# castorini/howl

Hardware: AMD Instinct MI355X
Metric: utterances/sec/node (res8 end-to-end training step, 1s@16kHz, 40-mel) (higher is better)
Workload: dtype f32; 1 GPU; res8 training step (frontend+fwd+xent+bwd+AdamW), 512 x 1 s utterances per GPU, 12 labels -- BASELINE configs[2] per-GPU share: res8 GSC-12, 512 x 1 s per GPU (4096 over 8); global_batch=512, samples_per_utterance=16000, labels=12, parallelism=single, frontend=eval

## Files before the change

### howl_amd/csrc/res8.hip

```cpp
#include "howl_common.hip.h"
#include "../../include/howl_hip.h"

namespace {

struct HowlPtrs6 {
    float* p[6];
};
constexpr int MAX_WINDOWS = 64;
struct HowlWinRows {
    int lo[MAX_WINDOWS], hi[MAX_WINDOWS];
};
struct HowlBnBuffers {
    float* running_mean;
    float* running_var;
    long long* num_batches;
};
struct BnFold {
    const float* part;
    int nparts;
    double count;
    float* stats_out;
    HowlBnBuffers bn;
};

// ... 1646 lines not shown
#pragma unroll
        for (int nt = 0; nt < 3; ++nt) {
            const int tap = 4 * ks + g, c = 16 * nt + n;
            bw[ks][nt] = (tap < 9 && c < NMAP) ? w0[c * 9 + tap] : 0.0f;
        }
    int aoff[3];
#pragma unroll
    for (int ks = 0; ks < 3; ++ks) {
        const int tap = min(4 * ks + g, 8);
        aoff[ks] = (tap / 3) * pitch + tap % 3 + (n & 7) + (n >> 3) * 3 * pitch;
    }
    for (int i = tid; i < 3 * pitch + 16; i += C0M_THREADS) tin[(T + 2) * pitch + i] = 0.0f;
    for (int item = blockIdx.x; item < B * slices; item += nconv) {
        const int b = item / slices, sl = item - b * slices;
        const int ph0 = (sl * H) / slices, ph1 = ((sl + 1) * H) / slices;
        __syncthreads();
        const int clip = b / nwin, wi = b - clip * nwin;
        const int t0 = EXACT ? wi * win_step : min(wi * win_step, win_last);
        load_feat_tile<EXACT>(tin, feat + (long)clip * sb + (long)t0 * st, 0, st, sm, 0, T, M, tid, C0M_THREADS, -t0, win_last - t0);
        __syncthreads();
        constexpr int NJ = 5 * NS;
        for (int u = wave; u < NJ * ((ph1 - ph0 + 1) / 2); u += C0M_THREADS / 64) {
            const int pp = u / NJ, j8 = u - NJ * pp;
            const float* rowp = tin + 3 * (ph0 + 2 * pp) * pitch + 8 * j8;
            {
                f32x4 acc[3][3];
#pragma unroll
                for (int tl = 0; tl < 3; ++tl)
#pragma unroll
                    for (int nt = 0; nt < 3; ++nt) acc[tl][nt] = {0.0f, 0.0f, 0.0f, 0.0f};
#pragma unroll
                for (int tl = 0; tl < 3; ++tl)
#pragma unroll
                    for (int ks = 0; ks < 3; ++ks) {
                        const float a = rowp[aoff[ks] + tl * pitch];
#pragma unroll
                        for (int nt = 0; nt < 3; ++nt)
                            acc[tl][nt] = __builtin_amdgcn_mfma_f32_16x16x4f32(a, bw[ks][nt], acc[tl][nt], 0, 0, 0);
                    }
                const int pw = 2 * j8 + (g & 1), ph = ph0 + 2 * pp + (g >> 1);
#pragma unroll
                for (int nt = 0; nt < 3; ++nt) {
                    float sum = 0.0f;
                    unsigned bits = 0;
#pragma unroll
                    for (int tl = 0; tl < 3; ++tl)
#pragma unroll
                        for (int r = 0; r < 4; ++r) {
                            const int rb = max(__float_as_int(acc[tl][nt][r]), 0);
                            sum += __int_as_float(rb);
                            bits |= min((unsigned)rb, 1u) << (4 * tl + r);
                        }
                    const int c = 16 * nt + n;
                    if (ph < ph1 && c < NMAP) {
                        const int strip = NS > 1 ? pw / PW : 0;
                        const size_t o = (((size_t)b * NS + strip) * NMAP + c) * P + (size_t)ph * PW + (pw - strip * PW);
                        s0[o] = sum * (1.0f / 12.0f);
                        if (mask0 != nullptr) mask0[o] = (unsigned short)bits;
                    }
                }
            }
        }
    }
}

constexpr int C0G_WAVES = 15, C0G_THREADS = 64 * C0G_WAVES, C0G_CPW = NMAP / C0G_WAVES;
static_assert(C0G_CPW * C0G_WAVES == NMAP, "channels split evenly over the waves");

__device__ __forceinline__ void load_patch(float (&x)[5][6], const float* tin, int pitch, int ph, int pw) {
    const float* base = tin + 3 * ph * pitch + 4 * pw;
#pragma unroll
    for (int r = 0; r < 5; ++r) {
        const float4 a = *reinterpret_cast<const float4*>(base + r * pitch);
        const float2 c = *reinterpret_cast<const float2*>(base + r * pitch + 4);
        x[r][0] = a.x, x[r][1] = a.y, x[r][2] = a.z, x[r][3] = a.w, x[r][4] = c.x, x[r][5] = c.y;
    }
}

template <int NS = 1, bool EXACT = false>
__global__ __launch_bounds__(C0G_THREADS) void conv0_wgrad_valu_kernel(const float* __restrict__ feat, long sb, long st, long sm,
                                                                      const unsigned short* __restrict__ mask0,
                                                                      const float* __restrict__ ga, const float* __restrict__ gb,
                                                                      float* __restrict__ part, int B, int T, int M, int H,
                                                                      int slices, StripGeom sg, int t_total) {
    HIP_DYNAMIC_SHARED(float, lds)
    float* tin = lds;
    const int tid = threadIdx.x, lane = tid & 63;
    const int wave = __builtin_amdgcn_readfirstlane(tid >> 6);
    const int pitch = M + 4;
    const int P = H * PW;
    float acc[C0G_CPW][9];
#pragma unroll
    for (int j = 0; j < C0G_CPW; ++j)
#pragma unroll
        for (int t = 0; t < 9; ++t) acc[j][t] = 0.0f;
    const int nrs = EXACT ? sg.nr : 1;
    for (int item = blockIdx.x; item < B * nrs * NS * slices; item += gridDim.x) {
        const int vb = item / slices, sl = item - vb * slices;
        const int vq = NS > 1 ? vb / NS : vb, strip = NS > 1 ? vb - vq * NS : 0;
        const int b = EXACT ? vq / nrs : vq, rs = EXACT ? vq - b * nrs : 0;
        const int Pv = (EXACT && rs == nrs - 1) ? sg.hv_last * PW : P;
        const int cell0 = (sl * Pv) / slices, cell1 = ((sl + 1) * Pv) / slices;
        __syncthreads();
        if constexpr (EXACT)
            load_feat_tile<true>(tin, feat + (long)rs * T * st, sb, st, sm, b, T, M, tid, C0G_THREADS, -rs * T, t_total - rs * T);
        else
            load_feat_tile(tin, feat, sb, st, sm, b, T, M, tid, C0G_THREADS);
        __syncthreads();
        const float* gab = ga + ((size_t)vb * NMAP + C0G_CPW * wave) * P;
        const float* gbb = gb != nullptr ? gb + ((size_t)vb * NMAP + C0G_CPW * wave) * P : nullptr;
        const unsigned short* mb = mask0 + ((size_t)vb * NMAP + C0G_CPW * wave) * P;
        for (int cb = cell0; cb < cell1; cb += 64) {
            const int cell = cb + lane;
            const bool valid = cell < cell1;
            const unsigned cc = (unsigned)(valid ? cell : cell1 - 1);
            float gv[C0G_CPW];
            unsigned mv[C0G_CPW];
#pragma unroll
            for (int j = 0; j < C0G_CPW; ++j) {
                const unsigned o = (unsigned)(j * P) + cc;
                gv[j] = gab[o] + (gbb != nullptr ? gbb[o] : 0.0f);
                mv[j] = mb[o];
            }
            const int ph = (int)cc / PW, pw = (int)cc - ph * PW;
            float x[5][6];
            load_patch(x, tin, pitch, ph, pw + strip * PW);
#pragma unroll
            for (int j = 0; j < C0G_CPW; ++j) {
                const int gbits = valid ? __float_as_int(gv[j] * (1.0f / 12.0f)) : 0;
#pragma unroll
                for (int tl = 0; tl < 3; ++tl)
#pragma unroll
                    for (int fl = 0; fl < 4; ++fl) {
                        const int k = 4 * tl + fl;
                        const int sel = ((int)(mv[j] << (31 - k))) >> 31;
                        const float dy = __int_as_float(sel & gbits);
#pragma unroll
                        for (int tap = 0; tap < 9; ++tap) acc[j][tap] = fmaf(dy, x[tl + tap / 3][fl + tap % 3], acc[j][tap]);
                    }
            }
        }
    }
#pragma unroll
    for (int j = 0; j < C0G_CPW; ++j)
#pragma unroll
        for (int t = 0; t < 9; ++t) {
            const float v = wave_sum_rows(acc[j][t]);
            if (lane == 0) part[(size_t)blockIdx.x * NMAP * 9 + (C0G_CPW * wave + j) * 9 + t] = v;
        }
}

constexpr int HEAD_XC = 64;
constexpr int HEAD_THREADS = 768, HEAD_PARTS = 16;
__global__ __launch_bounds__(HEAD_THREADS) void head_fwd_kernel(const float* __restrict__ s6, const float* __restrict__ stats,
                                                       const float* __restrict__ wout, const float* __restrict__ bout,
                                                       float* __restrict__ pooled, float* __restrict__ logits, int B,
                                                       int P, int C, const long long* __restrict__ labels,
                                                       float* __restrict__ nll, float* __restrict__ dlogits,
                                                       float* __restrict__ dpool, float inv_batch,
                                                       const float* __restrict__ pool, int npg, int npg_used, BnFold fold,
                                                       int ns ) {
    __shared__ float lp[CP];
    __shared__ float ll[HEAD_XC], dl[HEAD_XC], lse_s;
    __shared__ float lst[2 * CP];
    __shared__ float lw[HEAD_XC * NMAP];
    __shared__ float lparts[HEAD_PARTS][CP];
    const int tid = threadIdx.x, lane = tid & 63, wave = tid >> 6;
    const bool w_in_lds = C <= HEAD_XC;
    if (w_in_lds)
        for (int i = tid; i < C * NMAP; i += HEAD_THREADS) lw[i] = wout[i];
    if (fold.part != nullptr) {
        const int c8 = lane >> 3;
        for (int w0 = wave; w0 < CP / 4; w0 += HEAD_THREADS / 64) {
            const int c = 4 * w0 + (c8 & 3);
            const double sm = fold_part_column(fold.part, part_stride(fold.nparts), fold.nparts, (c8 < 4 ? 0 : CP) + c, lane);
            const double q = __shfl_xor(sm, 32);
            if (c8 < 4 && (lane & 7) == 0) {
                const double mean = sm / fold.count;
                double var = q / fold.count - mean * mean;
                var = var < 0.0 ? 0.0 : var;
                const float fm = (c < NMAP) ? (float)mean : 0.0f;
                const float fr = (c < NMAP) ? (float)(1.0 / sqrt(var + (double)BN_EPS)) : 0.0f;
                lst[c] = fm;
                lst[CP + c] = fr;
                if (blockIdx.x == 0) {
                    fold.stats_out[c] = fm;
                    fold.stats_out[CP + c] = fr;
                    if (c < NMAP && fold.bn.running_mean != nullptr) {
                        const double unbiased = fold.count > 1.0 ? var * fold.count / (fold.count - 1.0) : var;
                        fold.bn.running_mean[c] = (1.0f - BN_MOMENTUM) * fold.bn.running_mean[c] + BN_MOMENTUM * (float)mean;
                        fold.bn.running_var[c] = (1.0f - BN_MOMENTUM) * fold.bn.running_var[c] + BN_MOMENTUM * (float)unbiased;
                    }
                    if (c == 0 && fold.bn.num_batches != nullptr) fold.bn.num_batches[0] += 1;
                }
            }
        }
    } else if (tid < 2 * CP) {
        lst[tid] = stats[tid];
    }
    __syncthreads();
    for (int b = blockIdx.x; b < B; b += gridDim.x) {
        __syncthreads();
        if (pool != nullptr) {
            const int nparts = ns * npg_used;
            const int pc = tid % CP, pk = tid / CP;
            float acc = 0.0f;
            for (int k0 = 0; k0 < nparts; k0 += HEAD_PARTS) {
                const int k = k0 + pk;
                if (k < nparts) {
                    const int sgi = k / npg_used, g = k - sgi * npg_used;
                    lparts[pk][pc] = pool[(((size_t)b * ns + sgi) * npg + g) * CP + pc];
                }
                __syncthreads();
                if (tid < CP) {
                    const int n = nparts - k0 < HEAD_PARTS ? nparts - k0 : HEAD_PARTS;
                    for (int j = 0; j < n; ++j) acc += lparts[j][tid];
                }
                __syncthreads();
            }
            if (tid < CP) {
                const float v = tid < NMAP ? (acc / (float)P - lst[tid]) * lst[CP + tid] : 0.0f;
                lp[tid] = v;
                pooled[(size_t)b * CP + tid] = v;
            }
        } else if (wave < 4)
        for (int c0 = wave; c0 < CP; c0 += 12) {
            float a8[3][8];
#pragma unroll
            for (int u = 0; u < 3; ++u) {
                const int c = c0 + 4 * u < NMAP ? c0 + 4 * u : NMAP - 1;
                const float* src = s6 + ((size_t)b * NMAP + c) * P;
#pragma unroll
                for (int j = 0; j < 8; ++j) a8[u][j] = src[min(lane + 64 * j, P - 1)];
            }
#pragma unroll
            for (int u = 0; u < 3; ++u) {
                const int c = c0 + 4 * u;
#pragma unroll
                for (int j = 0; j < 8; ++j) a8[u][j] = (lane + 64 * j < P) ? fabsf(a8[u][j]) : 0.0f;
                float acc = ((a8[u][0] + a8[u][1]) + (a8[u][2] + a8[u][3])) + ((a8[u][4] + a8[u][5]) + (a8[u][6] + a8[u][7]));
                acc = wave_sum(acc);
                const float v = c < NMAP ? (acc / (float)P - lst[c]) * lst[CP + c] : 0.0f;
                if (lane == 0 && c < CP) {
                    lp[c] = v;
                    pooled[(size_t)b * CP + c] = v;
                }
            }
        }
        __syncthreads();
        for (int k = tid; k < C; k += HEAD_THREADS) {
            float acc = bout[k];
            if (w_in_lds)
                for (int c = 0; c < NMAP; ++c) acc = fmaf(lw[k * NMAP + c], lp[c], acc);
            else
                for (int c = 0; c < NMAP; ++c) acc = fmaf(wout[k * NMAP + c], lp[c], acc);
            logits[(size_t)b * C + k] = acc;
            if (labels != nullptr) ll[k] = acc;
        }
        if (labels == nullptr) continue;
        __syncthreads();
        const int y = (int)labels[b];
        if (tid == 0) {
            float mx = ll[0];
            for (int k = 1; k < C; ++k) mx = fmaxf(mx, ll[k]);
            float se = 0.0f;
            for (int k = 0; k < C; ++k) se += expf(ll[k] - mx);
            const float lse = mx + logf(se);
            lse_s = lse;
            nll[b] = lse - ll[y];
        }
        __syncthreads();
        if (tid < C) {
            const float d = (expf(ll[tid] - lse_s) - (tid == y ? 1.0f : 0.0f)) * inv_batch;
            dl[tid] = d;
            dlogits[(size_t)b * C + tid] = d;
        }
        __syncthreads();
        if (tid < CP) {
            float acc = 0.0f;
            if (tid < NMAP)
                for (int k = 0; k < C; ++k) acc = fmaf(dl[k], lw[k * NMAP + tid], acc);
            dpool[(size_t)b * CP + tid] = acc;
        }
    }
}

__global__ __launch_bounds__(256) void head_fwd_windows_kernel(const float* __restrict__ s6, const float* __restrict__ stats,
                                                               const float* __restrict__ wout, const float* __restrict__ bout,
                                                               float* __restrict__ logits, int B, int nwin, int Hw,
                                                               HowlWinRows rows, float inv_count, int C, int ns) {
    __shared__ float lp[CP];
    const int tid = threadIdx.x, lane = tid & 63, wave = tid >> 6;
    const int Pw = Hw * PW;
    for (int b = blockIdx.x; b < B; b += gridDim.x) {
        __syncthreads();
        for (int c = wave; c < CP; c += 4) {
            float acc = 0.0f;
            if (c < NMAP) {
                for (int w = 0; w < nwin * ns; ++w) {
                    const float* src = s6 + ((size_t)(b * nwin * ns + w) * NMAP + c) * Pw;
                    for (int i = rows.lo[w / ns] * PW + lane; i < rows.hi[w / ns] * PW; i += 64) acc += fabsf(src[i]);
                }
            }
            acc = wave_sum(acc);
            if (lane == 0) lp[c] = c < NMAP ? (acc * inv_count - stats[c]) * stats[CP + c] : 0.0f;
        }
        __syncthreads();
        for (int k = tid; k < C; k += 256) {
            float acc = bout[k];
            for (int c = 0; c < NMAP; ++c) acc = fmaf(wout[k * NMAP + c], lp[c], acc);
            logits[(size_t)b * C + k] = acc;
        }
    }
}

__global__ void head_bwd_pool_kernel(const float* __restrict__ dlogits, const float* __restrict__ wout,
                                     float* __restrict__ dpool, int B, int C) {
    const int idx = blockIdx.x * blockDim.x + threadIdx.x;
    if (idx >= B * CP) return;
    const int b = idx / CP, c = idx - b * CP;
    float acc = 0.0f;
    if (c < NMAP)
        for (int k = 0; k < C; ++k) acc = fmaf(dlogits[(size_t)b * C + k], wout[k * NMAP + c], acc);
    dpool[idx] = acc;
}

__global__ __launch_bounds__(1024) void head_bwd_param_kernel(const float* __restrict__ dlogits,
                                                              const float* __restrict__ pooled,
                                                              const float* __restrict__ dpool, float* __restrict__ dwout,
                                                              float* __restrict__ dbout, float* __restrict__ m12, int B,
                                                              int C, int P, const float* __restrict__ nll,
                                                              float* __restrict__ loss) {
    __shared__ double red[2][16][64];
    if ((int)blockIdx.x == C + 1) {
        double acc = 0.0;
        for (int b = threadIdx.x; b < B; b += 1024) acc += (double)nll[b];
        acc = wave_sum_d(acc);
        if ((threadIdx.x & 63) == 0) red[0][threadIdx.x >> 6][0] = acc;
        __syncthreads();
        if (threadIdx.x == 0) {
            double tot = 0.0;
            for (int w = 0; w < 16; ++w) tot += red[0][w][0];
            loss[0] = (float)(tot / (double)B);
        }
        return;
    }
    const int k = blockIdx.x, c = threadIdx.x & 63, bg = threadIdx.x >> 6;
    double a0 = 0.0, a1 = 0.0;
    constexpr int HR = 16;
    const int cc = c < CP ? c : CP - 1;
    if (k < C) {
        for (int b = bg; b < B; b += 16 * HR) {
            float d[HR], pv[HR];
#pragma unroll
            for (int j = 0; j < HR; ++j) {
                const int bb = b + 16 * j < B ? b + 16 * j : B - 1;
                d[j] = dlogits[(size_t)bb * C + k];
                pv[j] = pooled[(size_t)bb * CP + cc];
            }
#pragma unroll
            for (int j = 0; j < HR; ++j) {
                const bool ok = b + 16 * j < B;
                a1 += ok ? (double)d[j] : 0.0;
                a0 += (ok && c < CP) ? (double)d[j] * (double)pv[j] : 0.0;
            }
        }
    } else if (c < CP) {
        for (int b = bg; b < B; b += 16 * HR) {
            float d[HR], pv[HR];
#pragma unroll
            for (int j = 0; j < HR; ++j) {
                const int bb = b + 16 * j < B ? b + 16 * j : B - 1;
                d[j] = dpool[(size_t)bb * CP + c];
                pv[j] = pooled[(size_t)bb * CP + c];
            }
#pragma unroll
            for (int j = 0; j < HR; ++j) {
                const bool ok = b + 16 * j < B;
                a0 += ok ? (double)d[j] : 0.0;
                a1 += ok ? (double)d[j] * (double)pv[j] : 0.0;
            }
        }
    }
    red[0][bg][c] = a0;
    red[1][bg][c] = a1;
    __syncthreads();
    if (bg != 0) return;
    double s0 = 0.0, s1 = 0.0;
    for (int g = 0; g < 16; ++g) {
        s0 += red[0][g][c];
        s1 += red[1][g][c];
    }
    if (k < C) {
        if (c < NMAP) dwout[k * NMAP + c] = (float)s0;
        if (c == 0) dbout[k] = (float)s1;
    } else if (c < CP) {
        const double n = (double)B * (double)P;
        m12[c] = (float)(s0 / n);
        m12[CP + c] = (float)(s1 / n);
    }
}

__global__ __launch_bounds__(1024) void xent_kernel(const float* __restrict__ logits, const long long* __restrict__ labels,
                                                    int B, int C, float* __restrict__ loss, float* __restrict__ dlogits) {
    __shared__ double red[16];
    double acc = 0.0;
    const float invB = 1.0f / (float)B;
    constexpr int XC = 32;
    for (int b = threadIdx.x; b < B; b += 1024) {
        const float* row = logits + (size_t)b * C;
        const int y = (int)labels[b];
        if (C <= XC) {
            float v[XC];
#pragma unroll
            for (int k = 0; k < XC; ++k) v[k] = row[k < C ? k : C - 1];
            float mx = v[0];
#pragma unroll
            for (int k = 1; k < XC; ++k) mx = k < C ? fmaxf(mx, v[k]) : mx;
            float se = 0.0f;
#pragma unroll
            for (int k = 0; k < XC; ++k) se += k < C ? expf(v[k] - mx) : 0.0f;
            const float lse = mx + logf(se);
            float vy = v[0];
#pragma unroll
            for (int k = 1; k < XC; ++k) vy = k == y ? v[k] : vy;
            acc += (double)(lse - vy);
            if (dlogits != nullptr) {
#pragma unroll
                for (int k = 0; k < XC; ++k)
                    if (k < C) dlogits[(size_t)b * C + k] = (expf(v[k] - lse) - (k == y ? 1.0f : 0.0f)) * invB;
            }
            continue;
        }
        float mx = row[0];
        for (int k = 1; k < C; ++k) mx = fmaxf(mx, row[k]);
        float se = 0.0f;
        for (int k = 0; k < C; ++k) se += expf(row[k] - mx);
        const float lse = mx + logf(se);
        acc += (double)(lse - row[y]);
        if (dlogits != nullptr)
            for (int k = 0; k < C; ++k)
                dlogits[(size_t)b * C + k] = (expf(row[k] - lse) - (k == y ? 1.0f : 0.0f)) * invB;
    }
    acc = wave_sum_d(acc);
    if ((threadIdx.x & 63) == 0) red[threadIdx.x >> 6] = acc;
    __syncthreads();
    if (threadIdx.x == 0) {
        double tot = 0.0;
        for (int w = 0; w < 16; ++w) tot += red[w];
        loss[0] = (float)(tot / (double)B);
    }
}

__global__ void adamw_kernel(float* __restrict__ p, const float* __restrict__ g, float* __restrict__ m,
                             float* __restrict__ v, size_t n, HowlAdamWCoef c) {
    for (size_t i = (size_t)blockIdx.x * blockDim.x + threadIdx.x; i < n; i += (size_t)gridDim.x * blockDim.x)
        howl_adamw_element(p, m, v, i, g[i], c);
}

}

namespace {

size_t conv0_tile_floats(int T, int M) { return (size_t)(T + 2) * (M + 4) + 3 * (M + 4) + 16; }
size_t conv_lds_bytes(int H, bool own_rows) {
    return (size_t)(3 * KSTEPS * 64 + tile_floats(H, own_rows) + 4 * CP + 12 * 2 * 16) * sizeof(float);
}
size_t wgrad_lds_bytes(int H) { return (size_t)(tile_floats_z(H) + tile_floats_x(H) + 6 * CP) * sizeof(float); }

struct Ws {
    float* wp_fwd;
    float* wp_bwd;
    float* part;
    float* part2;
    float* stats;
    float* m12;
    float* dpool;
    float* pool;
    float* bufa;
    float* bufb;
    float* dz;
    float* dz2;
    float* dsa;
    float* dsb;
    float* wpart;
    float* c0part;
};

size_t ws_layout(Ws* w, char* base, int B, int H, int G, int cus, size_t* fwd_eval_bytes) {
    size_t off = 0;
    auto take = [&](size_t floats) {
        float* p = base ? reinterpret_cast<float*>(base + off) : nullptr;
        off += ((floats * sizeof(float) + 255) / 256) * 256;
        return p;
    };
    const size_t act = (size_t)B * NMAP * H * PW;
    w->wp_fwd = take((size_t)6 * 3 * KSTEPS * 64);
    w->wp_bwd = take((size_t)6 * 3 * KSTEPS * 64);
    const int max_parts = G > cus ? G : cus;
    w->part = take((size_t)part_stride(max_parts) * 2 * CP);
    w->part2 = take((size_t)part_stride(max_parts) * 2 * CP);
    w->stats = take((size_t)6 * 2 * CP);
    w->m12 = take(2 * CP);
    w->dpool = take((size_t)B * CP);
    w->pool = take((size_t)B * 16 * CP);
    *fwd_eval_bytes = off;
    w->bufa = take(act);
    w->bufb = take(act);
    w->dz = take(act);
    w->dz2 = take(act);
    w->dsa = take(act);
    w->dsb = take(act);
    w->wpart = take((size_t)6 * G * CP * WNCOL);
    w->c0part = take((size_t)max_parts * NMAP * 9);
    return off;
}

int mel_strips(int M) { return M == 40 ? 1 : (M == 80 ? 2 : 0); }
int even_grid(int g, int strips) { return strips > 1 ? ((g & ~1) > 2 ? (g & ~1) : 2) : g; }
int launch_blocks(int nblk, int per_group) { return 8 * per_group * ((nblk + 7) / 8); }
int conv_slices(int nblk, int H, int budget) {
    const int ntiles = (H * PW + 15) / 16;
    for (int sl = 4; sl > 1; sl >>= 1)
        if (nblk * sl <= budget && 4 * sl <= ntiles) return sl;
    return 1;
}
void pair_slices(int nblk, int H, int cus, int* sd, int* sw) {
    const int ntiles = (H * PW + 15) / 16;
    const int opts[3][2] = {{4, 2}, {2, 2}, {2, 1}};
    *sd = *sw = 1;
    for (const auto& o : opts)
        if (nblk * (o[0] + o[1]) <= cus && 4 * o[0] <= ntiles) {
            *sd = o[0];
            *sw = o[1];
            return;
        }
}
int conv0_slices(int B, int cus) {
    const int sl = cus / (B > 0 ? B : 1);
    return sl < 1 ? 1 : (sl > 8 ? 8 : sl);
}
bool env_off(const char* name) {
    const char* e = getenv(name);
    return e != nullptr && e[0] == '0';
}

constexpr int WIN_H = MAX_H, WIN_MARGIN = 7, WIN_STEP = WIN_H - 2 * WIN_MARGIN;
int long_windows(int H) { return H <= WIN_H ? 1 : (H - WIN_H + WIN_STEP - 1) / WIN_STEP + 1; }

struct Res8Plan {
    int B, T, M, ns, nr, Hs, hv_last, Bv, halo;
    StripGeom sg;
    int P, Pt;
    bool slicing, merged, fused;
    int G, SL;
    size_t lds_conv;
    int Bw, Tw, S0, G0, c0_nwin, c0_step, c0_last;
    bool c0_exact;
    size_t lds_conv0;
    int Gh, SD, SW, ew_grid;
    bool fold_in_pair;
    size_t wpart_stride, lds_wgrad, lds_pair;
    int S0w, G0w;
    size_t lds_conv0w;
    size_t saved_floats, train_bytes, eval_bytes;
    size_t long_map_bytes, long_bytes;
    Ws ws;
};

void plan_launches(Res8Plan& p, bool slice_conv0, char* ws_base) {
    const int cus = howl_num_cus(), H = p.Hs;
    p.P = H * PW;
    p.Pt = (p.T / 3) * PW * p.ns;
    p.saved_floats = (size_t)p.Bv * NMAP * p.P;
    p.slicing = !env_off("HOWL_RES8_SLICES");
    p.merged = !env_off("HOWL_RES8_BWD_PAIR");
    p.fused = p.halo != 0 || !env_off("HOWL_RES8_BWD_FUSED");

    p.G = even_grid(p.Bv < cus ? p.Bv : cus, p.ns);
    p.SL = p.halo == 0 && p.slicing ? conv_slices(p.G, H, cus) : 1;
    p.lds_conv = conv_lds_bytes(H, p.halo == 2);
    p.S0 = slice_conv0 && p.slicing ? conv0_slices(p.Bw, cus) : 1;
    p.G0 = p.Bw * p.S0 < 2 * cus ? p.Bw * p.S0 : 2 * cus;
    p.lds_conv0 = conv0_tile_floats(p.Tw, p.M) * sizeof(float);

    const int half = cus / 2 > 0 ? cus / 2 : 1;
    p.Gh = even_grid(p.Bv < half ? p.Bv : half, p.ns);
    p.SD = p.SW = 1;
    if (p.halo == 0 && p.slicing) pair_slices(p.Gh, H, cus, &p.SD, &p.SW);
    p.fold_in_pair = p.Gh * p.SD >= 64;
    p.wpart_stride = (size_t)p.Gh * CP * WNCOL;
    p.lds_wgrad = wgrad_lds_bytes(H);
    p.lds_pair = p.lds_conv > p.lds_wgrad ? p.lds_conv : p.lds_wgrad;
    const size_t quads = (p.saved_floats / 4 + BRB_THREADS - 1) / BRB_THREADS;
    p.ew_grid = quads < 1 ? 1 : (quads > (size_t)(2 * cus) ? 2 * cus : (int)quads);
    p.S0w = p.slicing ? conv0_slices(p.Bv, cus) : 1;
    p.G0w = p.Bv * p.S0w < cus ? p.Bv * p.S0w : cus;
    p.lds_conv0w = ((size_t)(p.Tw + 2) * (p.M + 4) + 16) * sizeof(float);

    p.train_bytes = ws_layout(&p.ws, ws_base, p.Bv, H, p.G, cus, &p.eval_bytes);
}

Res8Plan res8_plan(int B, int T, int M, void* ws = nullptr) {
    Res8Plan p{};
    const int H = T / 3;
    p.B = B, p.T = T, p.M = M;
    p.ns = mel_strips(M) > 0 ? mel_strips(M) : 1;
    p.nr = H <= MAX_H ? 1 : (H + MAX_H - 1) / MAX_H;
    p.Hs = (H + p.nr - 1) / p.nr;
    p.hv_last = H - (p.nr - 1) * p.Hs;
    p.Bv = B * p.nr * p.ns;
    p.halo = p.nr > 1 ? 2 : (p.ns > 1 ? 1 : 0);
    p.sg = StripGeom{p.nr, p.ns, p.hv_last};
    p.c0_exact = p.halo == 2;
    p.Bw = B * p.nr;
    p.Tw = p.c0_exact ? 3 * p.Hs : T;
    p.c0_nwin = p.c0_exact ? p.nr : 1;
    p.c0_step = p.c0_exact ? 3 * p.Hs : 0;
    p.c0_last = p.c0_exact ? T : 0;
    plan_launches(p, true, static_cast<char*>(ws));
    return p;
}

Res8Plan res8_long_plan(int B, int T, int M, void* ws = nullptr) {
    Res8Plan p{};
    const int H = T / 3, nw = long_windows(H);
    p.B = B, p.T = T, p.M = M;
    p.ns = mel_strips(M) > 0 ? mel_strips(M) : 1;
    p.nr = 1, p.Hs = p.hv_last = WIN_H;
    p.Bv = B * nw * p.ns;
    p.halo = p.ns > 1 ? 1 : 0;
    p.sg = StripGeom{1, 1, 0};
    p.Bw = B * nw;
    p.Tw = 3 * WIN_H + T % 3;
    p.c0_nwin = nw, p.c0_step = 3 * WIN_STEP, p.c0_last = 3 * (H - WIN_H);
    static_assert((6 * 2 * CP * sizeof(float)) % 256 == 0, "statistics block keeps the 256-byte alignment");
    p.long_map_bytes = ((size_t)p.Bv * NMAP * WIN_H * PW * sizeof(float) + 255) / 256 * 256;
    const size_t front = 3 * p.long_map_bytes + 6 * 2 * CP * sizeof(float) + 256;
    plan_launches(p, false, ws ? static_cast<char*>(ws) + front : nullptr);
    p.long_bytes = front + p.train_bytes;
    return p;
}

int check_workspace(const char* who, size_t have, size_t need) {
    if (have >= need) return HOWL_OK;
    howl_set_error("%s: workspace %zu < %zu bytes", who, have, need);
    return HOWL_E_WORKSPACE;
}
template <class T>
HowlPtrs6 ptrs6(T* const (&a)[6]) {
    HowlPtrs6 r;
    for (int i = 0; i < 6; ++i) r.p[i] = const_cast<float*>(a[i]);
    return r;
}
StageCfg plain_tile(const float* t) { return StageCfg{t, nullptr, nullptr, nullptr, nullptr, 0.0f, false, false, false}; }

template <auto Kernel>
void raise_lds_limit(size_t lds) {
    static thread_local size_t granted[16] = {};
    howl_raise_lds(reinterpret_cast<const void*>(Kernel), lds, granted, "res8 kernel");
}
template <int HALO>
StripGeom geom_arg(const Res8Plan& p) { return HALO == 2 ? p.sg : StripGeom{1, 1, 0}; }

struct Conv3x3Launch {
    StageCfg in;
    const float* in_stats = nullptr;
    const float* wp = nullptr;
    const float* res = nullptr;
    float* out = nullptr;
    const float* xs = nullptr;
    const float* xs_stats = nullptr;
    float* part = nullptr;
    float* pool = nullptr;
    BnFold fold{};
    BwdFold bfold{};
    WFold wf{nullptr, 0, nullptr};
};
template <int MODE, int SLICES, int HALO>
void launch_conv3x3_inst(const Res8Plan& p, hipStream_t stream, const Conv3x3Launch& a) {
    const int nblk = MODE == 0 ? p.G : p.Gh;
    raise_lds_limit<conv3x3_mfma_kernel<MODE, SLICES, HALO>>(p.lds_conv);
    hipLaunchKernelGGL((conv3x3_mfma_kernel<MODE, SLICES, HALO>), dim3(launch_blocks(nblk, SLICES)), dim3(CONV_THREADS), p.lds_conv,
                       stream, a.in, a.in_stats, a.wp, a.res, a.out, a.xs, a.xs_stats, a.part, a.pool, p.Bv, p.Hs, nblk, a.fold,
                       a.bfold, a.wf, geom_arg<HALO>(p));
}
template <int MODE>
void launch_conv3x3(const Res8Plan& p, hipStream_t stream, const Conv3x3Launch& a) {
    const int slices = MODE == 0 ? p.SL : p.SD;
    if (p.halo == 2)
        launch_conv3x3_inst<MODE, 1, 2>(p, stream, a);
    else if (p.halo == 1)
        launch_conv3x3_inst<MODE, 1, 1>(p, stream, a);
    else if (slices == 4)
        launch_conv3x3_inst<MODE, 4, 0>(p, stream, a);
    else if (slices == 2)
        launch_conv3x3_inst<MODE, 2, 0>(p, stream, a);
    else
        launch_conv3x3_inst<MODE, 1, 0>(p, stream, a);
}

struct BwdLayerLaunch {
    StageCfg zc;
    BwdFold bfold;
    const float* wp;
    float* dx;
    const float* xs;
    const float* xs_stats;
    float* spart;
    const float* s_prev;
    const float* in_stats;
    float* wpart;
    WFold wf;
};
template <int SD, int SW, int HALO>
void launch_pair_inst(const Res8Plan& p, hipStream_t stream, const BwdLayerLaunch& a) {
    raise_lds_limit<bwd_pair_kernel<SD, SW, HALO>>(p.lds_pair);
    hipLaunchKernelGGL((bwd_pair_kernel<SD, SW, HALO>), dim3(launch_blocks(p.Gh, SD + SW)), dim3(CONV_THREADS), p.lds_pair, stream, a.zc,
                       a.bfold, a.wp, a.dx, a.xs, a.xs_stats, a.spart, a.s_prev, a.in_stats, a.wpart, p.Bv, p.Hs, p.Gh, a.wf,
                       geom_arg<HALO>(p));
}
void launch_pair(const Res8Plan& p, hipStream_t stream, const BwdLayerLaunch& a) {
    if (p.halo == 2)
        launch_pair_inst<1, 1, 2>(p, stream, a);
    else if (p.halo == 1)
        launch_pair_inst<1, 1, 1>(p, stream, a);
    else if (p.SD == 4 && p.SW == 2)
        launch_pair_inst<4, 2, 0>(p, stream, a);
    else if (p.SD == 2 && p.SW == 2)
        launch_pair_inst<2, 2, 0>(p, stream, a);
    else if (p.SD == 2 && p.SW == 1)
        launch_pair_inst<2, 1, 0>(p, stream, a);
    else
        launch_pair_inst<1, 1, 0>(p, stream, a);
}
template <int SW, int HALO>
void launch_wgrad_inst(const Res8Plan& p, hipStream_t stream, const BwdLayerLaunch& a) {
    StageCfg zw = a.zc;
    zw.ds = nullptr;
    raise_lds_limit<wgrad_mfma_kernel<SW, HALO>>(p.lds_wgrad);
    hipLaunchKernelGGL((wgrad_mfma_kernel<SW, HALO>), dim3(launch_blocks(p.Gh, SW)), dim3(CONV_THREADS), p.lds_wgrad, stream,
                       WStage{zw, a.s_prev, false}, a.in_stats, a.bfold, a.wpart, p.Bv, p.Hs, p.Gh, geom_arg<HALO>(p));
}
void launch_wgrad(const Res8Plan& p, hipStream_t stream, const BwdLayerLaunch& a) {
    if (p.halo == 2)
        launch_wgrad_inst<1, 2>(p, stream, a);
    else if (p.halo == 1)
        launch_wgrad_inst<1, 1>(p, stream, a);
    else if (p.SW == 2)
        launch_wgrad_inst<2, 0>(p, stream, a);
    else
        launch_wgrad_inst<1, 0>(p, stream, a);
}

struct Feat {
    const float* x;
    long sb, st, sm;
};
template <int NS, bool EXACT>
void launch_conv0_fwd_inst(const Res8Plan& p, hipStream_t stream, const Feat& f, const HowlRes8Params* prm, float* s0,
                           unsigned short* mask0) {
    const int npack = (2 * 6 * PACK_ELEMS + C0M_THREADS - 1) / C0M_THREADS;
    hipLaunchKernelGGL((conv0_fwd_mfma_kernel<NS, EXACT>), dim3(p.G0 + npack), dim3(C0M_THREADS), p.lds_conv0, stream, f.x, f.sb, f.st,
                       f.sm, prm->conv0_w, s0, mask0, p.Bw, p.Tw, p.M, p.Hs, p.G0, ptrs6(prm->conv_w), p.ws.wp_fwd, p.ws.wp_bwd,
                       p.c0_nwin, p.c0_step, p.c0_last, p.S0);
}
void launch_conv0_fwd(const Res8Plan& p, hipStream_t stream, const Feat& f, const HowlRes8Params* prm, float* s0,
                      unsigned short* mask0) {
    if (p.c0_exact && p.ns == 2)
        launch_conv0_fwd_inst<2, true>(p, stream, f, prm, s0, mask0);
    else if (p.c0_exact)
        launch_conv0_fwd_inst<1, true>(p, stream, f, prm, s0, mask0);
    else if (p.ns == 2)
        launch_conv0_fwd_inst<2, false>(p, stream, f, prm, s0, mask0);
    else
        launch_conv0_fwd_inst<1, false>(p, stream, f, prm, s0, mask0);
}
template <int NS, bool EXACT>
void launch_conv0_wgrad_inst(const Res8Plan& p, hipStream_t stream, const Feat& f, const unsigned short* mask0, const float* g0) {
    hipLaunchKernelGGL((conv0_wgrad_valu_kernel<NS, EXACT>), dim3(p.G0w), dim3(C0G_THREADS), p.lds_conv0w, stream, f.x, f.sb, f.st, f.sm,
                       mask0, g0, (const float*)nullptr, p.ws.c0part, p.B, p.Tw, p.M, p.Hs, p.S0w, p.sg, p.T);
}
void launch_conv0_wgrad(const Res8Plan& p, hipStream_t stream, const Feat& f, const unsigned short* mask0, const float* g0) {
    if (p.c0_exact && p.ns == 2)
        launch_conv0_wgrad_inst<2, true>(p, stream, f, mask0, g0);
    else if (p.c0_exact)
        launch_conv0_wgrad_inst<1, true>(p, stream, f, mask0, g0);
    else if (p.ns == 2)
        launch_conv0_wgrad_inst<2, false>(p, stream, f, mask0, g0);
    else
        launch_conv0_wgrad_inst<1, false>(p, stream, f, mask0, g0);
}

int res8_fwd_impl(const HowlRes8Params* prm, const Feat& feat, int B, int T, int M, int C, int training, const HowlRes8Saved* sv,
                  float* logits, void* ws, size_t ws_bytes, const long long* labels, float* nll, float* dlogits, hipStream_t stream) {
    HOWL_REQUIRE(prm && feat.x && sv && logits && ws, "howl_res8_fwd: null pointer");
    HOWL_REQUIRE(labels == nullptr || (nll != nullptr && dlogits != nullptr && C <= HEAD_XC),
                 "howl_res8_fwd_xent: nll / dlogits missing or more than %d classes (C=%d)", HEAD_XC, C);
    HOWL_REQUIRE(mel_strips(M) > 0, "howl_res8_fwd: res8 pools (3,4) over 40 or 80 mel bins; got M=%d", M);
    HOWL_REQUIRE(B >= 1 && T / 3 >= 1, "howl_res8_fwd: B=%d T=%d unsupported (T >= 3)", B, T);
    HOWL_REQUIRE(C >= 1, "howl_res8_fwd: C must be positive");
    const Res8Plan p = res8_plan(B, T, M, ws);
    HOWL_REQUIRE(p.hv_last >= 1 && p.nr <= MAX_ROW_STRIPS, "howl_res8_fwd: T=%d frames unsupported (%d row strips)", T, p.nr);
    if (int rc = check_workspace("howl_res8_fwd", ws_bytes, training ? p.train_bytes : p.eval_bytes)) return rc;
    const Ws& w = p.ws;
    if (!training)
        hipLaunchKernelGGL(bn_eval_stats_kernel, dim3(6), dim3(64), 0, stream, ptrs6(prm->bn_running_mean), ptrs6(prm->bn_running_var),
                           sv->bn_stats);
    {
        HowlProfScope prof("conv0_fwd", stream);
        launch_conv0_fwd(p, stream, feat, prm, sv->s[0], sv->mask0);
    }
    const double count = (double)B * (double)p.Pt;
    const auto fold_of = [&](int layer, float* part) {
        return BnFold{part, p.G * p.SL, count, sv->bn_stats + (size_t)(layer - 1) * 2 * CP,
                      HowlBnBuffers{prm->bn_running_mean[layer - 1], prm->bn_running_var[layer - 1], prm->bn_num_batches[layer - 1]}};
    };
    for (int i = 1; i <= 6; ++i) {
        Conv3x3Launch a;
        a.in = plain_tile(sv->s[i - 1]);
        a.wp = w.wp_fwd + (size_t)(i - 1) * 3 * KSTEPS * 64;
        a.res = (i % 2) == 0 ? sv->s[i - 2] : nullptr;
        a.out = sv->s[i];
        a.part = training ? ((i & 1) ? w.part : w.part2) : nullptr;
        a.pool = i == 6 ? w.pool : nullptr;
        if (i > 1 && training)
            a.fold = fold_of(i - 1, (i & 1) ? w.part2 : w.part);
        else if (i > 1)
            a.in_stats = sv->bn_stats + (size_t)(i - 2) * 2 * CP;
        HowlProfScope prof("conv3x3_fwd", stream);
        launch_conv3x3<0>(p, stream, a);
    }
    const int groups = 4 * p.SL;
    hipLaunchKernelGGL(head_fwd_kernel, dim3(B < 1024 ? B : 1024), dim3(HEAD_THREADS), 0, stream, sv->s[6],
                       sv->bn_stats + (size_t)5 * 2 * CP, prm->out_w, prm->out_b, sv->pooled, logits, B, p.Pt, C, labels, nll, dlogits,
                       w.dpool, 1.0f / (float)B, (const float*)w.pool, groups, groups < (p.P + 15) / 16 ? groups : (p.P + 15) / 16,
                       training ? fold_of(6, w.part2) : BnFold{}, p.nr * p.ns);
    HOWL_CHECK_LAUNCH("howl_res8_fwd");
    return HOWL_OK;
}

int res8_bwd_impl(const HowlRes8Params* prm, const Feat& feat, int B, int T, int M, int C, const HowlRes8Saved* sv, const float* dlogits,
                  const HowlRes8Grads* gr, void* ws, size_t ws_bytes, int part, const float* nll, float* loss, hipStream_t stream,
                  const HowlAdamW* adamw = nullptr) {
    HOWL_REQUIRE(prm && feat.x && sv && dlogits && gr && ws, "howl_res8_bwd: null pointer");
    HOWL_REQUIRE(adamw == nullptr || (part == 0 && adamw->p && adamw->g && adamw->m && adamw->v && adamw->n >= 1 && adamw->step >= 1),
                 "howl_res8_bwd: HowlAdamW needs the whole pass (part 0) and complete buffers");
    HOWL_REQUIRE(part >= 0 && part <= 2, "howl_res8_bwd_part: part must be 0 (all), 1 or 2");
    const bool run_layers = part != 2, run_conv0 = part != 1;
    HOWL_REQUIRE(mel_strips(M) > 0, "howl_res8_bwd: M must be 40 or 80 (got %d)", M);
    HOWL_REQUIRE(B >= 1 && T / 3 >= 1, "howl_res8_bwd: B=%d T=%d unsupported", B, T);
    const Res8Plan p = res8_plan(B, T, M, ws);
    HOWL_REQUIRE(p.hv_last >= 1 && p.nr <= MAX_ROW_STRIPS, "howl_res8_bwd: T=%d frames unsupported (%d row strips)", T, p.nr);
    if (int rc = check_workspace("howl_res8_bwd", ws_bytes, p.train_bytes)) return rc;
    HOWL_REQUIRE(p.saved_floats / 2 < (size_t)1 << 31, "howl_res8_bwd: B=%d too large for the 32-bit element index of the elementwise pass", B);
    const Ws& w = p.ws;
    const double count = (double)B * (double)p.Pt;

    if (run_layers) {
        if (nll == nullptr)
            hipLaunchKernelGGL(head_bwd_pool_kernel, dim3((B * CP + 255) / 256), dim3(256), 0, stream, dlogits, prm->out_w, w.dpool,
                               B, C);
        hipLaunchKernelGGL(head_bwd_param_kernel, dim3(C + (nll != nullptr ? 2 : 1)), dim3(1024), 0, stream, dlogits, sv->pooled,
                           w.dpool, gr->out_w, gr->out_b, w.m12, B, C, p.Pt, nll, loss);
    }
    float* dx_cur = nullptr;
    float* dx_next = w.bufa;
    float* ds_prev = nullptr;
    float* ds_free = w.dsa;
    for (int i = 6; i >= 1; --i) {
        const bool even = (i % 2) == 0;
        const float* stats_i = sv->bn_stats + (size_t)(i - 1) * 2 * CP;
        float* ds_out = even ? ds_free : nullptr;
        float* dz = even ? w.dz : w.dz2;
        float* part_in = p.fused ? ((i & 1) ? w.part2 : w.part) : w.part;
        float* part_out = p.fused ? ((i & 1) ? w.part : w.part2) : w.part;
        BwdLayerLaunch a;
        a.bfold = BwdFold{stats_i, w.m12, i == 6 ? (const float*)nullptr : (const float*)part_in, p.Gh * p.SD, count};
        a.zc = plain_tile(dz);
        if (p.fused)
            a.zc = StageCfg{dx_cur, sv->s[i], even ? (const float*)ds_prev : (const float*)nullptr, ds_out, w.dpool,
                            1.0f / (float)p.Pt, true, even, false};
        else if (run_layers)
            hipLaunchKernelGGL(bn_relu_bwd_kernel, dim3(p.ew_grid), dim3(BRB_THREADS), 0, stream, (const float*)dx_cur, w.dpool, sv->s[i],
                               stats_i, w.m12, a.bfold.part, p.Gh * p.SD, count, even ? (const float*)ds_prev : (const float*)nullptr,
                               even ? 1 : 0, ds_out, dz, B, p.P);
        if (even) {
            float* t = ds_prev ? ds_prev : w.dsb;
            ds_prev = ds_out;
            ds_free = t;
        }
        const bool need_stats = i > 1;
        a.s_prev = sv->s[i - 1];
        a.in_stats = need_stats ? sv->bn_stats + (size_t)(i - 2) * 2 * CP : nullptr;
        a.wp = w.wp_bwd + (size_t)(i - 1) * 3 * KSTEPS * 64;
        a.dx = dx_next;
        a.xs = need_stats ? sv->s[i - 1] : (const float*)ds_prev;
        a.xs_stats = a.in_stats;
        a.spart = need_stats ? part_out : nullptr;
        a.wpart = w.wpart + (size_t)(i - 1) * p.wpart_stride;
        a.wf = (p.fold_in_pair && i < 6) ? WFold{w.wpart + (size_t)i * p.wpart_stride, p.Gh, gr->conv_w[i]} : WFold{nullptr, 0, nullptr};
        if (!run_layers) {
        } else if (p.merged) {
            HowlProfScope prof("bwd_pair", stream);
            launch_pair(p, stream, a);
        } else {
            {
                HowlProfScope prof("conv3x3_dgrad", stream);
                Conv3x3Launch d;
                d.in = a.zc, d.wp = a.wp, d.out = a.dx, d.xs = a.xs, d.xs_stats = a.xs_stats, d.part = a.spart;
                d.bfold = a.bfold, d.wf = a.wf;
                launch_conv3x3<1>(p, stream, d);
            }
            HowlProfScope prof("wgrad", stream);
            launch_wgrad(p, stream, a);
        }
        dx_cur = dx_next;
        dx_next = (dx_next == w.bufa) ? w.bufb : w.bufa;
    }
    HOWL_REQUIRE(sv->mask0 != nullptr, "howl_res8_bwd: saved->mask0 is required");
    const HowlPtrs6 gw = ptrs6(gr->conv_w);
    const RowsAdamW no_opt{nullptr, nullptr, nullptr, nullptr, HowlAdamWCoef{}, 0, 0, 0};
    const auto reduce_rows = [&](int cols, int first, int skip, int nrows, const RowsAdamW& opt) {
        hipLaunchKernelGGL(reduce_rows_all_kernel, dim3((cols + 63) / 64, nrows + (opt.on ? 1 : 0)), dim3(1024), 0, stream,
                           (const float*)w.wpart, p.wpart_stride, p.Gh, gw, (const float*)w.c0part, p.G0w, gr->conv0_w, first, skip,
                           nrows, opt);
    };
    if (part == 1)
        reduce_rows(CP * WNCOL, 0, 0, p.fold_in_pair ? 1 : 6, no_opt);
    if (run_conv0) {
        {
            HowlProfScope prof("conv0_wgrad", stream);
            launch_conv0_wgrad(p, stream, feat, sv->mask0, dx_cur);
        }
        if (part == 0) {
            RowsAdamW opt = no_opt;
            bool own_launch = adamw != nullptr;
            if (adamw != nullptr && getenv("HOWL_NO_FOLD_ADAMW") == nullptr) {
                const float* g0 = adamw->g;
                bool flat = gr->conv0_w == g0 && gr->out_b == gr->out_w + (size_t)NMAP * C &&
                            adamw->n == (size_t)NMAP * 9 + (size_t)6 * NMAP * NMAP * 9 + (size_t)NMAP * C + (size_t)C &&
                            gr->out_w == g0 + (size_t)NMAP * 9 + (size_t)6 * NMAP * NMAP * 9;
                for (int i = 0; i < 6; ++i) flat = flat && gr->conv_w[i] == g0 + (size_t)NMAP * 9 + (size_t)i * NMAP * NMAP * 9;
                if (flat) {
                    opt = RowsAdamW{adamw->p, g0, adamw->m, adamw->v,
                                    howl_adamw_coef(adamw->lr, adamw->beta1, adamw->beta2, adamw->eps, adamw->weight_decay, adamw->step,
                                                    adamw->grad_scale),
                                    (long)((p.fold_in_pair ? gr->conv_w[1] : gr->out_w) - g0), (long)adamw->n, 1};
                    own_launch = false;
                }
            }
            reduce_rows(CP * WNCOL, 0, p.fold_in_pair ? 5 : 0, p.fold_in_pair ? 2 : 7, opt);
            if (own_launch) {
                const int rc = howl_adamw_step(adamw->p, adamw->g, adamw->m, adamw->v, adamw->n, adamw->lr, adamw->beta1, adamw->beta2,
                                               adamw->eps, adamw->weight_decay, adamw->step, adamw->grad_scale, stream);
                if (rc != HOWL_OK) return rc;
            }
        } else {
            reduce_rows(NMAP * 9, 6, 0, 1, no_opt);
        }
    }
    HOWL_CHECK_LAUNCH("howl_res8_bwd");
    return HOWL_OK;
}

}

extern "C" {

size_t howl_res8_workspace_bytes(int B, int T) { return res8_plan(B, T, 40).train_bytes; }
size_t howl_res8_workspace_bytes_mels(int B, int T, int M) { return res8_plan(B, T, M).train_bytes; }
size_t howl_res8_saved_floats(int B, int T, int M) { return res8_plan(B, T, M).saved_floats; }
size_t howl_res8_eval_workspace_bytes_mels(int B, int T, int M) { return res8_plan(B, T, M).eval_bytes; }
int howl_res8_row_strips(int T) { return res8_plan(1, T, 40).nr; }

int howl_res8_fwd(const HowlRes8Params* prm, const float* feat, long sb, long st, long sm, int B, int T, int M, int C,
                  int training, const HowlRes8Saved* sv, float* logits, void* ws, size_t ws_bytes, hipStream_t stream) {
    return res8_fwd_impl(prm, Feat{feat, sb, st, sm}, B, T, M, C, training, sv, logits, ws, ws_bytes, nullptr, nullptr, nullptr, stream);
}

size_t howl_res8_long_workspace_bytes(int B, int T) { return res8_long_plan(B, T, 40).long_bytes; }
size_t howl_res8_long_workspace_bytes_mels(int B, int T, int M) { return res8_long_plan(B, T, M).long_bytes; }

int howl_res8_fwd_long(const HowlRes8Params* prm, const float* feat, long sb, long st, long sm, int B, int T, int M, int C,
                       float* logits, void* ws, size_t ws_bytes, hipStream_t stream) {
    HOWL_REQUIRE(prm && feat && logits && ws, "howl_res8_fwd_long: null pointer");
    HOWL_REQUIRE(mel_strips(M) > 0, "howl_res8_fwd_long: res8 pools (3,4) over 40 or 80 mel bins; got M=%d", M);
    const int H = T / 3;
    HOWL_REQUIRE(B >= 1 && H > WIN_H && C >= 1, "howl_res8_fwd_long: for T > 83 frames (got B=%d T=%d); shorter inputs use howl_res8_fwd", B, T);
    const int nw = long_windows(H);
// ... 90 lines not shown
```

Before: 473,500 utterances/sec.

## Process one utterance per wave in the res8 head training kernel

Adds a head_step_kernel for training that assigns one utterance to each wavefront, twelve per block, instead of one utterance per 768-thread block. The pooled partial sums are prefetched into registers before the BN-stat fold and LDS weight load, so those loads overlap the fold, and wave-local syncs replace block barriers. This cuts the number of blocks and barrier stalls in the small head stage, but every block still recomputes the BN fold. The old kernel remains the fallback and can be selected with an environment variable.

```diff
diff --git a/howl_amd/csrc/res8.hip b/howl_amd/csrc/res8.hip
--- a/howl_amd/csrc/res8.hip
+++ b/howl_amd/csrc/res8.hip
@@ -1822,6 +1822,35 @@
 
 constexpr int HEAD_XC = 64;
 constexpr int HEAD_THREADS = 768, HEAD_PARTS = 16;
+
+__device__ __forceinline__ void head_fold_stats(const BnFold& fold, float* lst, int lane, int wave) {
+    const int c8 = lane >> 3;
+    for (int w0 = wave; w0 < CP / 4; w0 += HEAD_THREADS / 64) {
+        const int c = 4 * w0 + (c8 & 3);
+        const double sm = fold_part_column(fold.part, part_stride(fold.nparts), fold.nparts, (c8 < 4 ? 0 : CP) + c, lane);
+        const double q = __shfl_xor(sm, 32);
+        if (c8 < 4 && (lane & 7) == 0) {
+            const double mean = sm / fold.count;
+            double var = q / fold.count - mean * mean;
+            var = var < 0.0 ? 0.0 : var;
+            const float fm = (c < NMAP) ? (float)mean : 0.0f;
+            const float fr = (c < NMAP) ? (float)(1.0 / sqrt(var + (double)BN_EPS)) : 0.0f;
+            lst[c] = fm;
+            lst[CP + c] = fr;
+            if (blockIdx.x == 0) {
+                fold.stats_out[c] = fm;
+                fold.stats_out[CP + c] = fr;
+                if (c < NMAP && fold.bn.running_mean != nullptr) {
+                    const double unbiased = fold.count > 1.0 ? var * fold.count / (fold.count - 1.0) : var;
+                    fold.bn.running_mean[c] = (1.0f - BN_MOMENTUM) * fold.bn.running_mean[c] + BN_MOMENTUM * (float)mean;
+                    fold.bn.running_var[c] = (1.0f - BN_MOMENTUM) * fold.bn.running_var[c] + BN_MOMENTUM * (float)unbiased;
+                }
+                if (c == 0 && fold.bn.num_batches != nullptr) fold.bn.num_batches[0] += 1;
+            }
+        }
+    }
+}
+
 __global__ __launch_bounds__(HEAD_THREADS) void head_fwd_kernel(const float* __restrict__ s6, const float* __restrict__ stats,
                                                        const float* __restrict__ wout, const float* __restrict__ bout,
                                                        float* __restrict__ pooled, float* __restrict__ logits, int B,
@@ -1840,31 +1869,7 @@
     if (w_in_lds)
         for (int i = tid; i < C * NMAP; i += HEAD_THREADS) lw[i] = wout[i];
     if (fold.part != nullptr) {
-        const int c8 = lane >> 3;
-        for (int w0 = wave; w0 < CP / 4; w0 += HEAD_THREADS / 64) {
-            const int c = 4 * w0 + (c8 & 3);
-            const double sm = fold_part_column(fold.part, part_stride(fold.nparts), fold.nparts, (c8 < 4 ? 0 : CP) + c, lane);
-            const double q = __shfl_xor(sm, 32);
-            if (c8 < 4 && (lane & 7) == 0) {
-                const double mean = sm / fold.count;
-                double var = q / fold.count - mean * mean;
-                var = var < 0.0 ? 0.0 : var;
-                const float fm = (c < NMAP) ? (float)mean : 0.0f;
-                const float fr = (c < NMAP) ? (float)(1.0 / sqrt(var + (double)BN_EPS)) : 0.0f;
-                lst[c] = fm;
-                lst[CP + c] = fr;
-                if (blockIdx.x == 0) {
-                    fold.stats_out[c] = fm;
-                    fold.stats_out[CP + c] = fr;
-                    if (c < NMAP && fold.bn.running_mean != nullptr) {
-                        const double unbiased = fold.count > 1.0 ? var * fold.count / (fold.count - 1.0) : var;
-                        fold.bn.running_mean[c] = (1.0f - BN_MOMENTUM) * fold.bn.running_mean[c] + BN_MOMENTUM * (float)mean;
-                        fold.bn.running_var[c] = (1.0f - BN_MOMENTUM) * fold.bn.running_var[c] + BN_MOMENTUM * (float)unbiased;
-                    }
-                    if (c == 0 && fold.bn.num_batches != nullptr) fold.bn.num_batches[0] += 1;
-                }
-            }
-        }
+        head_fold_stats(fold, lst, lane, wave);
     } else if (tid < 2 * CP) {
         lst[tid] = stats[tid];
     }
@@ -1955,6 +1960,91 @@
     }
 }
 
+constexpr int HEAD_WAVES = HEAD_THREADS / 64;
+static_assert(HEAD_WAVES == CP / 4, "head_fold_stats: one quad of statistics columns per wave");
+__global__ __launch_bounds__(HEAD_THREADS) void head_step_kernel(const float* __restrict__ wout, const float* __restrict__ bout,
+                                                        float* __restrict__ pooled, float* __restrict__ logits, int B, int P,
+                                                        int C, const long long* __restrict__ labels, float* __restrict__ nll,
+                                                        float* __restrict__ dlogits, float* __restrict__ dpool, float inv_batch,
+                                                        const float* __restrict__ pool, int npg, int npg_used, BnFold fold,
+                                                        int ns) {
+    __shared__ float lst[2 * CP];
+    __shared__ float lw[HEAD_XC * NMAP];
+    __shared__ float lp[HEAD_WAVES][CP], ll[HEAD_WAVES][HEAD_XC], le[HEAD_WAVES][HEAD_XC], dl[HEAD_WAVES][HEAD_XC];
+    const int tid = threadIdx.x, lane = tid & 63, wave = tid >> 6;
+    const int b = blockIdx.x * HEAD_WAVES + wave;
+    const int bb = b < B ? b : B - 1;
+    const int pc = lane < CP ? lane : CP - 1, kc = lane < C ? lane : C - 1;
+    const int nparts = ns * npg_used;
+
+    float pv[HEAD_PARTS];
+    {
+        int sgi = 0, g = 0;
+#pragma unroll
+        for (int j = 0; j < HEAD_PARTS; ++j) {
+            const bool in = j < nparts;
+            pv[j] = pool[(((size_t)bb * ns + (in ? sgi : 0)) * npg + (in ? g : 0)) * CP + pc];
+            if (++g == npg_used) g = 0, ++sgi;
+        }
+    }
+    const int y = (int)labels[bb];
+    const float bias = bout[kc];
+    for (int i = tid; i < C * NMAP; i += HEAD_THREADS) lw[i] = wout[i];
+    head_fold_stats(fold, lst, lane, wave);
+    __syncthreads();
+    if (b >= B) return;
+
+    float acc = 0.0f;
+#pragma unroll
+    for (int j = 0; j < HEAD_PARTS; ++j)
+        if (j < nparts) acc += pv[j];
+    for (int k0 = HEAD_PARTS; k0 < nparts; k0 += HEAD_PARTS) {
+        int sgi = k0 / npg_used, g = k0 - sgi * npg_used;
+#pragma unroll
+        for (int j = 0; j < HEAD_PARTS; ++j) {
+            const bool in = k0 + j < nparts;
+            pv[j] = pool[(((size_t)b * ns + (in ? sgi : 0)) * npg + (in ? g : 0)) * CP + pc];
+            if (++g == npg_used) g = 0, ++sgi;
+        }
+#pragma unroll
+        for (int j = 0; j < HEAD_PARTS; ++j)
+            if (k0 + j < nparts) acc += pv[j];
+    }
+    if (lane < CP) {
+        const float v = lane < NMAP ? (acc / (float)P - lst[lane]) * lst[CP + lane] : 0.0f;
+        lp[wave][lane] = v;
+        pooled[(size_t)b * CP + lane] = v;
+    }
+    wave_lds_sync();
+    float lg = bias;
+    for (int c = 0; c < NMAP; ++c) lg = fmaf(lw[kc * NMAP + c], lp[wave][c], lg);
+    if (lane < C) {
+        logits[(size_t)b * C + lane] = lg;
+        ll[wave][lane] = lg;
+    }
+    wave_lds_sync();
+    float mx = ll[wave][0];
+    for (int k = 1; k < C; ++k) mx = fmaxf(mx, ll[wave][k]);
+    if (lane < C) le[wave][lane] = expf(lg - mx);
+    wave_lds_sync();
+    float se = 0.0f;
+    for (int k = 0; k < C; ++k) se += le[wave][k];
+    const float lse = mx + logf(se);
+    if (lane == 0) nll[b] = lse - ll[wave][y];
+    if (lane < C) {
+        const float d = (expf(lg - lse) - (lane == y ? 1.0f : 0.0f)) * inv_batch;
+        dl[wave][lane] = d;
+        dlogits[(size_t)b * C + lane] = d;
+    }
+    wave_lds_sync();
+    if (lane < CP) {
+        float dp = 0.0f;
+        if (lane < NMAP)
+            for (int k = 0; k < C; ++k) dp = fmaf(dl[wave][k], lw[k * NMAP + lane], dp);
+        dpool[(size_t)b * CP + lane] = dp;
+    }
+}
+
 __global__ __launch_bounds__(256) void head_fwd_windows_kernel(const float* __restrict__ s6, const float* __restrict__ stats,
                                                                const float* __restrict__ wout, const float* __restrict__ bout,
                                                                float* __restrict__ logits, int B, int nwin, int Hw,
@@ -2222,7 +2312,7 @@
     int B, T, M, ns, nr, Hs, hv_last, Bv, halo;
     StripGeom sg;
     int P, Pt;
-    bool slicing, merged, fused;
+    bool slicing, merged, fused, head_waves;
     int G, SL;
     size_t lds_conv;
     int Bw, Tw, S0, G0, c0_nwin, c0_step, c0_last;
@@ -2246,6 +2336,7 @@
     p.slicing = !env_off("HOWL_RES8_SLICES");
     p.merged = !env_off("HOWL_RES8_BWD_PAIR");
     p.fused = p.halo != 0 || !env_off("HOWL_RES8_BWD_FUSED");
+    p.head_waves = !env_off("HOWL_RES8_HEAD_WAVES");
 
     p.G = even_grid(p.Bv < cus ? p.Bv : cus, p.ns);
     p.SL = p.halo == 0 && p.slicing ? conv_slices(p.G, H, cus) : 1;
@@ -2501,11 +2592,16 @@
         HowlProfScope prof("conv3x3_fwd", stream);
         launch_conv3x3<0>(p, stream, a);
     }
-    const int groups = 4 * p.SL;
-    hipLaunchKernelGGL(head_fwd_kernel, dim3(B < 1024 ? B : 1024), dim3(HEAD_THREADS), 0, stream, sv->s[6],
-                       sv->bn_stats + (size_t)5 * 2 * CP, prm->out_w, prm->out_b, sv->pooled, logits, B, p.Pt, C, labels, nll, dlogits,
-                       w.dpool, 1.0f / (float)B, (const float*)w.pool, groups, groups < (p.P + 15) / 16 ? groups : (p.P + 15) / 16,
-                       training ? fold_of(6, w.part2) : BnFold{}, p.nr * p.ns);
+    const int groups = 4 * p.SL, groups_used = groups < (p.P + 15) / 16 ? groups : (p.P + 15) / 16;
+    if (p.head_waves && training && labels != nullptr)
+        hipLaunchKernelGGL(head_step_kernel, dim3((B + HEAD_WAVES - 1) / HEAD_WAVES), dim3(HEAD_THREADS), 0, stream, prm->out_w,
+                           prm->out_b, sv->pooled, logits, B, p.Pt, C, labels, nll, dlogits, w.dpool, 1.0f / (float)B,
+                           (const float*)w.pool, groups, groups_used, fold_of(6, w.part2), p.nr * p.ns);
+    else
+        hipLaunchKernelGGL(head_fwd_kernel, dim3(B < 1024 ? B : 1024), dim3(HEAD_THREADS), 0, stream, sv->s[6],
+                           sv->bn_stats + (size_t)5 * 2 * CP, prm->out_w, prm->out_b, sv->pooled, logits, B, p.Pt, C, labels, nll,
+                           dlogits, w.dpool, 1.0f / (float)B, (const float*)w.pool, groups, groups_used,
+                           training ? fold_of(6, w.part2) : BnFold{}, p.nr * p.ns);
     HOWL_CHECK_LAUNCH("howl_res8_fwd");
     return HOWL_OK;
 }
```

New measurement: 476,500 utterances/sec, median of 6. Within noise of the previous version (+0.6%).
